# Kolkir/mono_slam_framework

Hardware: AMD Instinct MI355X
Metric: frame-pairs/sec (extract+match) (higher is better)
Workload: dtype u8; 1 GPU; ORB extract+match, 1280x720 pairs, 1024 pairs/GPU/step resident in HBM, ratio 0.60; pairs_per_gpu=1024, width=1280, height=720, synth_mode=0, overflow_pairs=0, ranks=1, rccl_ranks=0

## Files before the change

mono_slam_framework_amd/csrc/orb_kernels.hip:

```cpp
#include <type_traits>
#include "orb_pipeline.h"

#include <math.h>
#include <stdlib.h>
#include <string.h>

#include "orb_pattern.h"

namespace msf {

constexpr int SW = TW + 2, SH = TH + 2;
constexpr int kTileCandCap = TW * TH / 4;
constexpr int kTileY0 = kEdge;

constexpr uint32_t kStatusOverflow = 1u;

__constant__ __attribute__((aligned(16))) signed char c_pattern[1024];
__constant__ uint32_t c_disc[2 * kDiscTasks];

__device__ __forceinline__ __amdgpu_buffer_rsrc_t uniform_rsrc(const void* p, uint32_t bytes) {
  const unsigned long long v = (unsigned long long)p;
  const uint32_t lo = (uint32_t)__builtin_amdgcn_readfirstlane((int)(uint32_t)v);
  const uint32_t hi = (uint32_t)__builtin_amdgcn_readfirstlane((int)(uint32_t)(v >> 32));
  return __builtin_amdgcn_make_buffer_rsrc((void*)(((unsigned long long)hi << 32) | lo), 0,
                                           (int)__builtin_amdgcn_readfirstlane((int)bytes), 0x00020000);
}
__device__ __forceinline__ uint32_t uniform_u32(uint32_t v) { return (uint32_t)__builtin_amdgcn_readfirstlane((int)v); }
__device__ __forceinline__ const uint8_t* level_ptr(const OrbGeometry& g, const FrameSrc& src,
                                                    const uint8_t* pyr, int fi, int l, int* pitch) {
  if (l == 0) {
    *pitch = src.row_stride;
    return fi < src.n_a ? src.a + (long long)fi * src.frame_stride
                        : src.b + (long long)(fi - src.n_a) * src.frame_stride;
  }
  *pitch = g.lv[l].pitch;
  return pyr + (long long)(src.slot0 + fi) * g.pyr_bytes + g.lv[l].pix_off;
}

typedef unsigned short us2_t __attribute__((ext_vector_type(2)));
__device__ __forceinline__ uint32_t udot2_u16(uint32_t a, uint32_t b, uint32_t c) {
  return __builtin_amdgcn_udot2(__builtin_bit_cast(us2_t, a), __builtin_bit_cast(us2_t, b), c, false);
}

__device__ __forceinline__ uint32_t mad_u24(uint32_t a, uint32_t b, uint32_t c) {
  uint32_t r;
  asm("v_mad_u32_u24 %0, %1, %2, %3" : "=v"(r) : "v"(a), "v"(b), "v"(c));
  return r;
}

__device__ __forceinline__ uint32_t mad_u24_s(uint32_t a, uint32_t b_uniform, uint32_t c) {
  uint32_t r;
  asm("v_mad_u32_u24 %0, %1, %2, %3" : "=v"(r) : "v"(a), "s"(b_uniform), "v"(c));
  return r;
}

constexpr int kResizeMaxRows = 16;
template <bool SHARED>
__global__ __launch_bounds__(256) void k_resize(OrbGeometry g, FrameSrc src, uint8_t* pyr,
                                                const uint32_t* __restrict__ tab, int l, int rth, int lds_rows,
                                                uint32_t magic_n16, uint32_t magic_groups) {
  extern __shared__ __attribute__((aligned(16))) uint8_t smem[];
  uint32_t* ysh = reinterpret_cast<uint32_t*>(smem);
  uint8_t* rt = smem + 4 * kResizeMaxRows * 2;
  const int fi = blockIdx.y;
  const OrbLevelInfo L = g.lv[l];
  const int sh = g.lv[l - 1].h, sw16 = (g.lv[l - 1].w + 16 + 15) & ~15;
  int spitch;
  const uint8_t* s = level_ptr(g, src, pyr, fi, l - 1, &spitch);
  uint8_t* d = pyr + (long long)(src.slot0 + fi) * g.pyr_bytes + L.pix_off;
  const int groups = (L.w + 3) >> 2;
  const uint4* xsel = reinterpret_cast<const uint4*>(tab + L.tab_off);
  const uint4* xwxp = xsel + groups;
  const uint4* xoff = xwxp + groups;
  const uint32_t* ytab = reinterpret_cast<const uint32_t*>(xoff + groups);
  const int Y0 = blockIdx.x * rth, tid = threadIdx.x, nthr = blockDim.x;
  const int ylast = min(Y0 + rth, L.h) - 1;
  const int sy0 = ytab[Y0] & 0xFFFF;
  const int nrow = min((int)(ytab[ylast] & 0xFFFF) + 2 - sy0, lds_rows);
  const int n16 = sw16 >> 4, n4 = sw16 >> 2, rows = ylast - Y0 + 1;
  const int rowb = 4 * n4;
  if (tid < kResizeMaxRows) {
    const int y = Y0 + min(tid, rows - 1);
    const uint32_t yt = ytab[y];
    const uint32_t step1 = (tid > 0 && tid < rows && (yt & 0xFFFF) == (ytab[y - 1] & 0xFFFF) + 1u) ? 0x80000000u : 0u;
    ysh[2 * tid] = (uint32_t)(((int)(yt & 0xFFFF) - sy0) * rowb);
    ysh[2 * tid + 1] = (yt >> 16) | step1;
  }
  const int rgs = (rows + 3) >> 2, ntask = rgs * groups;
  int i = tid;
  int rg = magic_groups ? (int)__umulhi((uint32_t)min(i, ntask - 1), magic_groups) : min(i, ntask - 1);
  int gq = min(i, ntask - 1) - rg * groups;
  uint4 qs = xsel[gq], qw = xwxp[gq], qo = xoff[gq];
  for (int i = tid; i < nrow * n16; i += nthr) {
    const int r = (int)__umulhi((uint32_t)i, magic_n16), c = i - r * n16;
    const int gx = 16 * c, gy = sy0 + r;
    uint4 v = make_uint4(0u, 0u, 0u, 0u);
    if (gy < sh && gx + 16 <= spitch) v = *reinterpret_cast<const uint4*>(s + (long long)gy * spitch + gx);
    reinterpret_cast<uint4*>(rt)[i] = v;
  }
  __syncthreads();
  for (; i < ntask; i += nthr) {
    const int x4 = 4 * gq, ry0 = 4 * rg;
    const uint32_t sel[4] = {qs.x, qs.y, qs.z, qs.w}, wxp[4] = {qw.x, qw.y, qw.z, qw.w};
    const uint32_t boff[4] = {qo.x + (uint32_t)rowb, (SHARED ? qo.x : qo.y) + (uint32_t)rowb,
                              (SHARED ? qo.x : qo.z) + (uint32_t)rowb, qo.w + (uint32_t)rowb};
    {
      const int in = min(i + nthr, ntask - 1);
      rg = magic_groups ? (int)__umulhi((uint32_t)in, magic_groups) : in;
      gq = in - rg * groups;
      qs = xsel[gq], qw = xwxp[gq], qo = xoff[gq];
    }
    const char* Tb = reinterpret_cast<const char*>(rt);
    uint8_t* dp = d + (long long)(Y0 + ry0) * L.pitch + x4;
    const uint4 ya = *reinterpret_cast<const uint4*>(ysh + 2 * ry0), yb = *reinterpret_cast<const uint4*>(ysh + 2 * ry0 + 4);
    const uint32_t yrb[4] = {ya.x, ya.z, yb.x, yb.z}, ywy[4] = {ya.y, ya.w, yb.y, yb.w};
    uint32_t hlow[4];
#pragma unroll
    for (int j = 0; j < 4; j++) {
      const char* pr = Tb + yrb[j];
      if (j == 0 || (int)ywy[j] >= 0) {
#pragma unroll
        for (int k = 0; k < 4; k++) {
          const uint32_t* pa = reinterpret_cast<const uint32_t*>(pr + boff[k] - rowb);
          hlow[k] = udot2_u16(__builtin_amdgcn_perm(pa[1], pa[0], sel[k]), wxp[k], 0u);
        }
      }
      const uint32_t wy1 = ywy[j], wy0 = 256u - wy1;
      uint32_t v[4];
#pragma unroll
      for (int k = 0; k < 4; k++) {
        const uint32_t* pc = reinterpret_cast<const uint32_t*>(pr + boff[k]);
        const uint32_t h1 = udot2_u16(__builtin_amdgcn_perm(pc[1], pc[0], sel[k]), wxp[k], 0u);
        v[k] = mad_u24(hlow[k], wy0, mad_u24(h1, wy1, 32768u));
        hlow[k] = h1;
      }
      const uint32_t packed = __builtin_amdgcn_perm(v[1], v[0], 0x0c0c0602u) | __builtin_amdgcn_perm(v[3], v[2], 0x06020c0cu);
      if (ry0 + j < rows) *reinterpret_cast<uint32_t*>(dp) = packed;
      dp += L.pitch;
    }
  }
}

constexpr int HX = 16, HY = 4;
constexpr int PW2 = TW + 2 * HX, PH2 = TH + 2 * HY;
constexpr int SCO = 4;
constexpr int GPR = TW / 4 + 2;
constexpr int kList1Cap = 2 * SW * SH;
static_assert(kFastT % 2 == 0, "prefilter constants assume an even FAST threshold (cv::ORB default 20)");

__device__ __forceinline__ uint32_t mbcnt64(unsigned long long m) {
  return __builtin_amdgcn_mbcnt_hi((uint32_t)(m >> 32), __builtin_amdgcn_mbcnt_lo((uint32_t)m, 0u));
}

template <bool BRIGHT, int PITCH = PW2>
__device__ __forceinline__ int fast_score_pol(const uint8_t* p, int tau) {
  constexpr int off[16] = {3 * PITCH + 0,  3 * PITCH + 1,  2 * PITCH + 2,  1 * PITCH + 3,  0 * PITCH + 3, -1 * PITCH + 3,
                           -2 * PITCH + 2, -3 * PITCH + 1, -3 * PITCH + 0, -3 * PITCH - 1, -2 * PITCH - 2, -1 * PITCH - 3,
                           0 * PITCH - 3,  1 * PITCH - 3,  2 * PITCH - 2,  3 * PITCH - 1};
  int q[16];
// ... 1244 lines not shown
                                                     const uint32_t* __restrict__ s1_cnt, uint4* s1) {
  const int fi = blockIdx.y, slot = src.slot0 + fi, lane = threadIdx.x & 63;
  const int u = blockIdx.x * 4 + (threadIdx.x >> 6);
  if (u >= hw.base[g.nlevels]) return;
  int l = 0;
#pragma unroll
  for (int i = 1; i < kOrbLevels; i++)
    if (i < g.nlevels && u >= hw.base[i]) l = i;
  const OrbLevelInfo L = g.lv[l];
  const uint32_t kept = min(s1_cnt[slot * kOrbLevels + l], (uint32_t)kS1Cap);
  uint4* out = s1 + (long long)slot * g.s1_total + L.s1_off;
  int pitch;
  const uint8_t* img = level_ptr(g, src, pyr, fi, l, &pitch);
  const uint32_t step = 64u * (uint32_t)hw.n[l];
  for (uint32_t i = 64u * (uint32_t)(u - hw.base[l]) + lane; i < kept; i += step) {
    const uint32_t key = out[i].x;
    out[i].y = __float_as_uint(harris_at(img, pitch, key & 0xFFFF, key >> 16));
  }
}

constexpr int kSelCap = kKpCap;
__global__ __launch_bounds__(256) void k_select(OrbGeometry g, int slot0, const uint32_t* s1_cnt, const uint4* s1,
                                                msf_keypoint* kp, uint32_t* kp_cnt, uint32_t* status) {
  __shared__ uint4 kept[kSelCap];
  constexpr int kRespCap = 4096;
  __shared__ __attribute__((aligned(16))) float resp[kRespCap];
  __shared__ __attribute__((aligned(16))) uint32_t keys[kSelCap];
  __shared__ uint32_t nkept;
  const int slot = slot0 + blockIdx.x, tid = threadIdx.x;
  msf_keypoint* out = kp + (long long)slot * kKpCap;
  uint32_t base = 0;
  bool overflow = false;
  for (int l = 0; l < g.nlevels; l++) {
    const OrbLevelInfo L = g.lv[l];
    const uint32_t n = s1_cnt[slot * kOrbLevels + l];
    const uint4* in = s1 + (long long)slot * g.s1_total + L.s1_off;
    const uint32_t keep = (uint32_t)L.quota;
    if (tid == 0) nkept = 0;
    const bool staged = n > keep && n <= (uint32_t)kRespCap;
    const uint32_t n4 = (n + 3) >> 2;
    if (staged)
      for (uint32_t i = tid; i < 4 * n4; i += 256) resp[i] = i < n ? __uint_as_float(in[i].y) : -INFINITY;
    __syncthreads();
    for (uint32_t i = tid; i < n; i += 256) {
      const uint4 e = in[i];
      bool k = true;
      if (n > keep) {
        const float v = __uint_as_float(e.y);
        uint32_t greater = 0;
        if (staged) {
          const float4* r4 = reinterpret_cast<const float4*>(resp);
          for (uint32_t j = 0; j < n4; j++) {
            const float4 r = r4[j];
            greater += (uint32_t)(r.x > v) + (uint32_t)(r.y > v) + (uint32_t)(r.z > v) + (uint32_t)(r.w > v);
          }
        } else {
          for (uint32_t j = 0; j < n; j++) greater += (__uint_as_float(in[j].y) > v) ? 1u : 0u;
        }
        k = greater < keep;
      }
      if (k) {
        const uint32_t q = atomicAdd(&nkept, 1u);
        if (q < (uint32_t)kSelCap) kept[q] = e;
      }
    }
    __syncthreads();
    uint32_t m = nkept;
    if (m > (uint32_t)kSelCap) { overflow = true; m = kSelCap; }
    if (base + m > (uint32_t)kKpCap) { overflow = true; m = kKpCap - base; }
    const uint32_t m4 = (m + 3) >> 2;
    for (uint32_t i = tid; i < 4 * m4; i += 256) keys[i] = i < m ? kept[i].x : 0xFFFFFFFFu;
    __syncthreads();
    for (uint32_t i = tid; i < m; i += 256) {
      const uint4 e = kept[i];
      uint32_t rank = 0;
      const uint4* k4 = reinterpret_cast<const uint4*>(keys);
      for (uint32_t j = 0; j < m4; j++) {
        const uint4 kk = k4[j];
        rank += (uint32_t)(kk.x < e.x) + (uint32_t)(kk.y < e.x) + (uint32_t)(kk.z < e.x) + (uint32_t)(kk.w < e.x);
      }
      msf_keypoint k;
      k.lx = e.x & 0xFFFF;
      k.ly = e.x >> 16;
      k.x = (float)k.lx * L.scale;
      k.y = (float)k.ly * L.scale;
      k.response = __uint_as_float(e.y);
      k.angle = -1.f;
      k.octave = l;
      k.fast_score = (int)e.z;
      out[base + rank] = k;
    }
    base += m;
    __syncthreads();
  }
  if (tid == 0) {
    kp_cnt[slot] = base;
    if (overflow) atomicOr(&status[slot], kStatusOverflow);
  }
}

__device__ __forceinline__ float fast_atan2_deg(float y, float x) {
  const float k = (float)(180.0 / 3.14159265358979323846);
  const float p1 = 0.9997878412794807f * k, p3 = -0.3258083974640975f * k, p5 = 0.1555786518463281f * k,
              p7 = -0.04432655554792128f * k;
  const float ax = fabsf(x), ay = fabsf(y);
  float a, c, c2;
  if (ax >= ay) {
    c = ay / (ax + (float)2.2204460492503131e-16);
    c2 = c * c;
    a = (((p7 * c2 + p5) * c2 + p3) * c2 + p1) * c;
  } else {
    c = ax / (ay + (float)2.2204460492503131e-16);
    c2 = c * c;
    a = 90.f - (((p7 * c2 + p5) * c2 + p3) * c2 + p1) * c;
  }
  if (x < 0) a = 180.f - a;
  if (y < 0) a = 360.f - a;
  return a;
}

__device__ __forceinline__ void det_sincosf(float t, float* s, float* c) {
  const double x = (double)t;
  const int k = (int)(x * 6.36619772367581382433e-01 + 0.5);
  const double kd = (double)k;
  const double r = (x - kd * 1.57079632673412561417e+00) - kd * 6.07710050650619224932e-11;
  const double z = r * r;
  double p = 1.58969099521155010221e-10;
  p = p * z + -2.50507602534068634195e-08;
  p = p * z + 2.75573137070700676789e-06;
  p = p * z + -1.98412698298579493134e-04;
  p = p * z + 8.33333333332248946124e-03;
  p = p * z + -1.66666666666666324348e-01;
  const double sr = r + (r * z) * p;
  double q = -1.13596475577881948265e-11;
  q = q * z + 2.08757232129817482790e-09;
  q = q * z + -2.75573143513906633035e-07;
  q = q * z + 2.48015872894767294178e-05;
  q = q * z + -1.38888888888741095749e-03;
  q = q * z + 4.16666666666666019037e-02;
  const double cr = (1.0 - 0.5 * z) + (z * z) * q;
  double sv, cv;
  switch (k & 3) {
    case 0: sv = sr; cv = cr; break;
    case 1: sv = cr; cv = -sr; break;
    case 2: sv = -sr; cv = -cr; break;
    default: sv = -cr; cv = sr; break;
  }
  *s = (float)sv;
  *c = (float)cv;
}

constexpr int PR = 22;
constexpr int PD = 2 * PR + 1;
constexpr int PP = 48;
constexpr int HP = 40;
constexpr int HC = 46;

template <bool HALF_UP, bool SUM256>
__global__ __launch_bounds__(256) void k_describe(OrbGeometry g, FrameSrc src, const uint8_t* pyr,
                                                  msf_keypoint* kp, const uint32_t* kp_cnt, uint8_t* desc) {
  __shared__ __attribute__((aligned(16))) uint8_t raw_s[4][PD * PP + 16];
  __shared__ __attribute__((aligned(16))) uint16_t hb_s[4][HP * HC];
  __shared__ uint32_t disc_s[2 * kDiscTasks];
  __shared__ __attribute__((aligned(16))) int pat_s[256];
  const int fi = blockIdx.y, slot = src.slot0 + fi;
  const int wave = __builtin_amdgcn_readfirstlane((int)(threadIdx.x >> 6)), lane = threadIdx.x & 63;
  for (int i = threadIdx.x; i < 2 * kDiscTasks; i += 256) disc_s[i] = c_disc[i];
  pat_s[threadIdx.x] = reinterpret_cast<const int*>(c_pattern)[threadIdx.x];
  __shared__ unsigned long long lvl_base_s[kOrbLevels];
  __shared__ int lvl_pitch_s[kOrbLevels];
  if (threadIdx.x < kOrbLevels) {
    int pt = 0;
    const uint8_t* bp = level_ptr(g, src, pyr, fi, threadIdx.x < g.nlevels ? (int)threadIdx.x : 0, &pt);
    lvl_base_s[threadIdx.x] = (unsigned long long)bp;
    lvl_pitch_s[threadIdx.x] = pt;
  }
  __syncthreads();
  const uint32_t count = min(kp_cnt[slot], (uint32_t)kKpCap);
  uint8_t* raw = raw_s[wave];
  uint16_t* hb = hb_s[wave];
  uint32_t* raw32 = reinterpret_cast<uint32_t*>(raw);
  constexpr int NPL = (PD * (PP / 4) + 63) / 64;
  const uint32_t kstride = gridDim.x * 4;
  uint32_t k = blockIdx.x * 4 + wave;
  uint32_t pre[NPL];
  int xo_pre = 0;
  auto meta = [&](uint32_t k_) -> uint3 {
    if (k_ >= count) return make_uint3(0u, 0u, 0u);
    const msf_keypoint* Kp = kp + (long long)slot * kKpCap + k_;
    return make_uint3((uint32_t)Kp->octave, (uint32_t)Kp->lx, (uint32_t)Kp->ly);
  };
  auto issue = [&](uint3 m) {
    const uint32_t lv = (uint32_t)__builtin_amdgcn_readfirstlane((int)m.x);
    const int mx = __builtin_amdgcn_readfirstlane((int)m.y), my = __builtin_amdgcn_readfirstlane((int)m.z);
    const uint32_t pitch_ = (uint32_t)__builtin_amdgcn_readfirstlane(lvl_pitch_s[lv]);
    const unsigned long long b64 = lvl_base_s[lv];
    const unsigned long long img_ = ((unsigned long long)(uint32_t)__builtin_amdgcn_readfirstlane((int)(b64 >> 32)) << 32) |
                                    (uint32_t)__builtin_amdgcn_readfirstlane((int)(uint32_t)b64);
    typedef const __attribute__((address_space(1))) uint8_t* gptr_t;
    const int ax = (mx - PR) & ~3;
    xo_pre = (mx - PR) - ax;
    gptr_t base = (gptr_t)(img_ + (unsigned long long)((long long)(my - PR) * (long long)pitch_ + ax));
    const uint32_t pm = pitch_ - (uint32_t)PP;
#pragma unroll
    for (int u = 0; u < NPL; u++) {
      const uint32_t i = (uint32_t)lane + 64u * (uint32_t)u;
      const uint32_t r = (i * 43691u) >> 19;
      const uint32_t off = mad_u24(r, pm, 4u * i);
      pre[u] = i < (uint32_t)(PD * (PP / 4)) ? *(const __attribute__((address_space(1))) uint32_t*)(base + off) : 0u;
    }
  };
  uint32_t* hb32 = reinterpret_cast<uint32_t*>(hb);
  const int blur_rl = (lane * 26) >> 8, blur_gq = lane - 10 * blur_rl;
  const int blur_rd = blur_rl * (2 * (PP / 4)) + blur_gq, blur_wr = blur_gq * (4 * (HC / 2)) + blur_rl;
  const bool blur_last = 18 + blur_rl < 23;
  const uint32_t samp_base = (uint32_t)(uintptr_t)(__attribute__((address_space(3))) uint16_t*)hb +
                             2u * (uint32_t)((PR - 3) * HC + (PR - 3)) - 2u * HC * 0x400000u - 2u * 0x4B400000u;
  uint3 m_cur = meta(k), m_next = meta(k + kstride);
  if (k < count) issue(m_cur);
  for (; k < count; k += kstride) {
    const bool active = true;
    msf_keypoint* K = kp + (long long)slot * kKpCap + k;
    const int l = (int)m_cur.x, cx = (int)m_cur.y, cy = (int)m_cur.z;
    (void)l; (void)cx; (void)cy;
    const int xo = xo_pre;
#pragma unroll
    for (int u = 0; u < NPL; u++) {
      const int i = lane + 64 * u;
      if (i < PD * (PP / 4)) raw32[i] = pre[u];
    }
    m_cur = m_next;
    if (k + kstride < count) issue(m_cur);
    m_next = meta(k + 2 * kstride);
    MSF_WAVE_SYNC();
    float angle = 0.f;
    if (active) {
      int m10 = 0, m01 = 0;
      {
        const int dw0 = 1 + ((xo + 2) >> 2);
        const uint32_t shf = (uint32_t)(xo + 2) & 3u;
#pragma unroll
        for (int it = 0; it < kDiscTasks / 64; it++) {
          const int t = it * 64 + lane;
          const int row = t >> 3, k = t & 7;
          const uint32_t* d = raw32 + (row + 7) * (PP / 4) + dw0 + k;
          const uint32_t pxw = __builtin_amdgcn_alignbyte(d[1], d[0], shf) ^ 0x80808080u;
          const uint32_t wu = disc_s[2 * t], wv = disc_s[2 * t + 1];
          m10 = __builtin_amdgcn_sdot4((int)pxw, (int)wu, m10, false);
          m01 = __builtin_amdgcn_sdot4((int)pxw, (int)wv, m01, false);
        }
      }
      m10 = (int)__builtin_amdgcn_readlane((int)wave_incl_scan((uint32_t)m10), 63);
      m01 = (int)__builtin_amdgcn_readlane((int)wave_incl_scan((uint32_t)m01), 63);
      angle = fast_atan2_deg((float)m01, (float)m10);
      {
        constexpr uint32_t T0 = 18, T1 = 34, T2 = SUM256 ? 48 : 49, T3 = SUM256 ? 56 : 55;
        constexpr uint32_t A0 = T0 | T1 << 8 | T2 << 16 | T3 << 24, B0 = T2 | T1 << 8 | T0 << 16;
        constexpr uint32_t A1 = T0 << 8 | T1 << 16 | T2 << 24, B1 = T3 | T2 << 8 | T1 << 16 | T0 << 24;
        constexpr uint32_t A2 = T0 << 16 | T1 << 24, B2 = T2 | T3 << 8 | T2 << 16 | T1 << 24, C2 = T0;
        constexpr uint32_t A3 = T0 << 24, B3 = T1 | T2 << 8 | T3 << 16 | T2 << 24, C3 = T1 | T0 << 8;
        auto row4 = [&](const uint32_t* d, uint32_t* o) {
          const uint32_t d0 = d[0], d1 = d[1], d2 = d[2], d3 = d[3];
          const uint32_t e0 = __builtin_amdgcn_alignbyte(d1, d0, xo), e1 = __builtin_amdgcn_alignbyte(d2, d1, xo);
          const uint32_t e2 = __builtin_amdgcn_alignbyte(d3, d2, xo);
          o[0] = __builtin_amdgcn_udot4(e0, A0, __builtin_amdgcn_udot4(e1, B0, 0u, false), false);
          o[1] = __builtin_amdgcn_udot4(e0, A1, __builtin_amdgcn_udot4(e1, B1, 0u, false), false);
          o[2] = __builtin_amdgcn_udot4(e0, A2, __builtin_amdgcn_udot4(e1, B2, __builtin_amdgcn_udot4(e2, C2, 0u, false), false), false);
          o[3] = __builtin_amdgcn_udot4(e0, A3, __builtin_amdgcn_udot4(e1, B3, __builtin_amdgcn_udot4(e2, C3, 0u, false), false), false);
        };
#pragma unroll
        for (int it = 0; it < 4; it++) {
          const uint32_t* d = raw32 + blur_rd + it * (12 * (PP / 4));
          uint32_t ou[4], ol[4];
          row4(d, ou);
          row4(d + PP / 4, ol);
          if (it < 3 || blur_last) {
            uint32_t* w = hb32 + blur_wr + it * 6;
#pragma unroll
            for (int j = 0; j < 4; j++) w[j * (HC / 2)] = ou[j] | (ol[j] << 16);
          }
        }
      }
    }
    MSF_WAVE_SYNC();
    if (active) {
      float a, b;
      float rad = angle;
      rad *= (float)(3.14159265358979323846 / 180.f);
      det_sincosf(rad, &b, &a);
      const int4 pk = *reinterpret_cast<const int4*>(&pat_s[lane * 4]);
      const int words[4] = {pk.x, pk.y, pk.z, pk.w};
      uint32_t nib = 0;
      constexpr uint32_t K2 = SUM256 ? 48 : 49, K3 = SUM256 ? 56 : 55;
      constexpr uint32_t P0 = 18u | 34u << 16, P1 = K2 | K3 << 16, P2 = K2 | 34u << 16, P3 = 18u;
#pragma unroll
      for (int t = 0; t < 4; t++) {
        uint32_t val[2];
#pragma unroll
        for (int e = 0; e < 2; e++) {
          const float px = (float)(signed char)(words[t] >> (16 * e));
          const float py = (float)(signed char)(words[t] >> (16 * e + 8));
          const uint32_t tx = __float_as_uint((px * a - py * b) + 12582912.f);
          const uint32_t ty = __float_as_uint((px * b + py * a) + 12582912.f);
          const uint32_t addr = mad_u24(tx, 2u * HC, (ty << 1) + samp_base);
          const __attribute__((address_space(3))) uint32_t* q =
              (const __attribute__((address_space(3))) uint32_t*)(uintptr_t)(addr & ~3u);
          const uint32_t sh = addr & 2u;
          const uint32_t d0 = q[0], d1 = q[1], d2 = q[2], d3 = q[3];
          const uint32_t w0 = __builtin_amdgcn_alignbyte(d1, d0, sh), w1 = __builtin_amdgcn_alignbyte(d2, d1, sh);
          const uint32_t w2 = __builtin_amdgcn_alignbyte(d3, d2, sh), w3 = __builtin_amdgcn_alignbyte(0u, d3, sh);
          const uint32_t sum = udot2_u16(w0, P0, udot2_u16(w1, P1, udot2_u16(w2, P2, udot2_u16(w3, P3, 0u))));
          const uint32_t r = HALF_UP ? (sum + 32768u) >> 16 : (sum + 0x7FFFu + ((sum >> 16) & 1u)) >> 16;
          val[e] = min(r, 255u);
        }
        nib |= (uint32_t)(val[0] < val[1]) << t;
      }
      const uint32_t hi = __shfl_down(nib, 1);
      if ((lane & 1) == 0) desc[((long long)slot * kKpCap + k) * 32 + (lane >> 1)] = (uint8_t)(nib | (hi << 4));
      if (lane == 0) K->angle = angle;
    }
    MSF_WAVE_SYNC();
  }
}

constexpr int kTrainChunk = 1024;
__global__ __launch_bounds__(256) void k_match(int n_pairs, const int32_t* slot_a, const int32_t* slot_b,
                                               const msf_keypoint* kp, const uint32_t* kp_cnt, const uint8_t* desc,
                                               const uint32_t* status, float ratio, msf_match* out, int cap,
                                               int32_t* n_out, int chunk, int slot_base, int max_slots) {
  __shared__ __attribute__((aligned(16))) unsigned long long train[kTrainChunk * 4];
  __shared__ uint32_t wave_cnt[4];
  __shared__ uint32_t running;
  const int pair = blockIdx.x, tid = threadIdx.x, lane = tid & 63, wave = tid >> 6;
  const int sa = slot_a ? slot_a[pair] : slot_base + pair;
  const int sb = slot_b ? slot_b[pair] : slot_base + n_pairs + pair;
  if (sa < 0 || sa >= max_slots || sb < 0 || sb >= max_slots || ((status[sa] | status[sb]) & kStatusOverflow)) {
    if (tid == 0) n_out[pair] = -1;
    return;
  }
  const uint32_t n1 = min(kp_cnt[sa], (uint32_t)kKpCap), n2 = min(kp_cnt[sb], (uint32_t)kKpCap);
  const unsigned long long* tsrc = reinterpret_cast<const unsigned long long*>(desc + (long long)sb * kKpCap * 32);
  if (tid == 0) running = 0;
  __syncthreads();
  const msf_keypoint* ka = kp + (long long)sa * kKpCap;
  const msf_keypoint* kb = kp + (long long)sb * kKpCap;
  msf_match* o = out + (long long)pair * cap;
  for (uint32_t q0 = 0; q0 < n1; q0 += 256) {
    const uint32_t q = q0 + tid;
    const bool have_q = q < n1;
    unsigned long long q0w = 0, q1w = 0, q2w = 0, q3w = 0;
    if (have_q) {
      const unsigned long long* qd =
          reinterpret_cast<const unsigned long long*>(desc + ((long long)sa * kKpCap + q) * 32);
      q0w = qd[0]; q1w = qd[1]; q2w = qd[2]; q3w = qd[3];
    }
    int d0 = 0x7fffffff, d1 = 0x7fffffff, i0 = -1;
    for (uint32_t t0 = 0; t0 < n2; t0 += chunk) {
      const uint32_t tn = min(n2 - t0, (uint32_t)chunk);
      __syncthreads();
      for (uint32_t i = tid; i < tn * 4; i += 256) train[i] = tsrc[(size_t)t0 * 4 + i];
      __syncthreads();
      if (have_q) {
        for (uint32_t t = 0; t < tn; t++) {
          const unsigned long long* tr = &train[t * 4];
          const int d = __popcll(q0w ^ tr[0]) + __popcll(q1w ^ tr[1]) + __popcll(q2w ^ tr[2]) + __popcll(q3w ^ tr[3]);
          if (d < d1) {
            if (d < d0) { d1 = d0; d0 = d; i0 = (int)(t0 + t); }
            else d1 = d;
          }
        }
      }
    }
    const bool pass = have_q && n2 >= 2 && ((float)d0 < ratio * (float)d1);
    const unsigned long long bal = __ballot(pass);
    const uint32_t before = __popcll(bal & ((1ull << lane) - 1ull));
    if (lane == 0) wave_cnt[wave] = __popcll(bal);
    __syncthreads();
    uint32_t off = running;
    for (int w = 0; w < wave; w++) off += wave_cnt[w];
    if (pass) {
      const uint32_t idx = off + before;
      if (idx < (uint32_t)cap) {
        msf_match m;
        m.x1 = (int)ka[q].x; m.y1 = (int)ka[q].y;
        m.x2 = (int)kb[i0].x; m.y2 = (int)kb[i0].y;
        o[idx] = m;
      }
    }
    __syncthreads();
    if (tid == 0) running += wave_cnt[0] + wave_cnt[1] + wave_cnt[2] + wave_cnt[3];
    __syncthreads();
  }
  if (tid == 0) n_out[pair] = (int32_t)running;
}

constexpr int kSplitBlocks = kKpCap / 64;
constexpr int kSplitMaxPairs = 128;
__global__ __launch_bounds__(256) void k_match_split(int n_pairs, const int32_t* slot_a, const int32_t* slot_b,
                                                     const msf_keypoint* kp, const uint32_t* kp_cnt,
                                                     const uint8_t* desc, const uint32_t* status, float ratio,
                                                     msf_match* out, int cap, int32_t* n_out, int chunk,
                                                     uint32_t* qres, uint32_t* done, int slot_base, int max_slots) {
  __shared__ __attribute__((aligned(16))) unsigned long long train[kTrainChunk * 4];
  __shared__ int part[3][4][64];
  __shared__ uint32_t wave_cnt[4];
  __shared__ uint32_t running, last_s;
  const int pair = blockIdx.y, qb = blockIdx.x, tid = threadIdx.x, lane = tid & 63, wave = tid >> 6;
  const int sa = slot_a ? slot_a[pair] : slot_base + pair;
  const int sb = slot_b ? slot_b[pair] : slot_base + n_pairs + pair;
  if (sa < 0 || sa >= max_slots || sb < 0 || sb >= max_slots || ((status[sa] | status[sb]) & kStatusOverflow)) {
    if (qb == 0 && tid == 0) n_out[pair] = -1;
    return;
  }
  const uint32_t n1 = min(kp_cnt[sa], (uint32_t)kKpCap), n2 = min(kp_cnt[sb], (uint32_t)kKpCap);
  const unsigned long long* tsrc = reinterpret_cast<const unsigned long long*>(desc + (long long)sb * kKpCap * 32);
  uint32_t* qr = qres + (long long)pair * kKpCap;
  const uint32_t q = (uint32_t)qb * 64u + lane;
  if ((uint32_t)qb * 64u < n1) {
    const bool have_q = q < n1;
    unsigned long long q0w = 0, q1w = 0, q2w = 0, q3w = 0;
    if (have_q) {
      const unsigned long long* qd = reinterpret_cast<const unsigned long long*>(desc + ((long long)sa * kKpCap + q) * 32);
      q0w = qd[0]; q1w = qd[1]; q2w = qd[2]; q3w = qd[3];
    }
    int d0 = 0x7fffffff, d1 = 0x7fffffff, i0 = 0x7fffffff;
    for (uint32_t t0 = 0; t0 < n2; t0 += chunk) {
      const uint32_t tn = min(n2 - t0, (uint32_t)chunk);
      __syncthreads();
      for (uint32_t i = tid; i < tn * 4; i += 256) train[i] = tsrc[(size_t)t0 * 4 + i];
      __syncthreads();
      const uint32_t ta = (tn * wave) >> 2, tb = (tn * (wave + 1)) >> 2;
      for (uint32_t t = ta; t < tb; t++) {
// ... 614 lines not shown
```

Baseline: 165,000 frame-pairs/sec.

## Compute descriptor patch row blur with MFMA int8 tiles and remap block-to-frame

```diff
diff --git a/mono_slam_framework_amd/csrc/orb_blur_tiles.h b/mono_slam_framework_amd/csrc/orb_blur_tiles.h
--- /dev/null
+++ b/mono_slam_framework_amd/csrc/orb_blur_tiles.h
@@ -0,0 +1,85 @@
+#pragma once
+#include <stdint.h>
+
+namespace msf {
+namespace blur_tiles {
+
+constexpr int kRawPitch = 48;
+constexpr int kRawRows = 45;
+constexpr int kRawRowsRead = 48;
+constexpr int kRawBytes = kRawRowsRead * kRawPitch + 16;
+constexpr int kFetchLoads = 9;
+constexpr int kFetchLanes = 60;
+constexpr int kHbCols = 40;
+constexpr int kHbRows = 46;
+constexpr int kHbPitch = 52;
+constexpr int kHbEntries = kHbCols * kHbPitch;
+constexpr int kTilesM = 3, kTilesN = 3;
+
+constexpr int tap(bool sum256, int j) {
+  const int k = j < 4 ? j : 6 - j;
+  return k == 0 ? 18 : k == 1 ? 34 : k == 2 ? (sum256 ? 48 : 49) : (sum256 ? 56 : 55);
+}
+constexpr int acc_init(bool sum256) { return 128 * (sum256 ? 256 : 257); }
+
+constexpr int fetch_lane(int lane) { return lane < kFetchLanes ? lane : kFetchLanes - 1; }
+constexpr int fetch_row(int lane) { return fetch_lane(lane) / 12; }
+constexpr int fetch_dword(int lane) { return fetch_lane(lane) % 12; }
+constexpr int raw_dword_of_load(int u, int lane) { return 60 * u + fetch_lane(lane); }
+
+constexpr int raw_col(int group, int byte) { return 16 * group + byte; }
+constexpr int a_byte_offset(int mt, int lane) { return (16 * mt + lane % 16) * kRawPitch + 16 * (lane / 16); }
+constexpr int b_weight(bool sum256, int nt, int lane, int byte) {
+  const int k = raw_col(lane / 16, byte), j = k - (16 * nt + lane % 16) - 2;
+  return k < kRawPitch && j >= 0 && j < 7 ? tap(sum256, j) : 0;
+}
+constexpr uint64_t tap_word(bool sum256) {
+  return (uint64_t)tap(sum256, 0) | (uint64_t)tap(sum256, 1) << 8 | (uint64_t)tap(sum256, 2) << 16 | (uint64_t)tap(sum256, 3) << 24 |
+         (uint64_t)tap(sum256, 4) << 32 | (uint64_t)tap(sum256, 5) << 40 | (uint64_t)tap(sum256, 6) << 48;
+}
+constexpr uint32_t b_dword(bool sum256, int nt, int lane, int d) {
+  const int j0 = 16 * (lane / 16) + 4 * d - (16 * nt + lane % 16) - 2;
+  return lane >= 48 || j0 <= -4 || j0 >= 7 ? 0u
+         : j0 >= 0 ? (uint32_t)(tap_word(sum256) >> (8 * j0)) : (uint32_t)(tap_word(sum256) << (8 * -j0));
+}
+
+constexpr int d_col(int nt, int lane) { return 16 * nt + lane % 16; }
+constexpr int d_row0(int mt, int lane) { return 16 * mt + 4 * (lane / 16); }
+constexpr int hb_store_dwords(int mt, int nt, int lane) {
+  return d_col(nt, lane) >= kHbCols ? 0 : d_row0(mt, lane) + 4 <= kHbRows ? 2 : d_row0(mt, lane) + 2 <= kHbRows ? 1 : 0;
+}
+constexpr int hb_store_byte_offset(int mt, int nt, int lane) { return 2 * (d_col(nt, lane) * kHbPitch + d_row0(mt, lane)); }
+constexpr uint32_t pack2(uint32_t lo, uint32_t hi) { return (lo & 0xFFFFu) | hi << 16; }
+
+constexpr int moment_dword(int t) { return (7 + t / 8) * (kRawPitch / 4) + 2 + t % 8; }
+constexpr int kSampleReach = 19;
+constexpr int samp_byte_offset(int ix, int iy) { return 2 * ((kSampleReach + ix) * kHbPitch + kSampleReach + iy); }
+
+inline void model_row_blur(bool sum256, const uint8_t* raw, uint16_t* hb) {
+  for (int mt = 0; mt < kTilesM; mt++)
+    for (int nt = 0; nt < kTilesN; nt++) {
+      int32_t acc[16][16];
+      for (int i = 0; i < 16; i++)
+        for (int n = 0; n < 16; n++) acc[i][n] = acc_init(sum256);
+      for (int la = 0; la < 64; la++)
+        for (int lb = 0; lb < 64; lb++) {
+          if (la / 16 != lb / 16) continue;
+          const uint8_t* a = raw + a_byte_offset(mt, la);
+          for (int j = 0; j < 16; j++)
+            acc[la % 16][lb % 16] += (int32_t)(int8_t)a[j] * (int32_t)(int8_t)(b_dword(sum256, nt, lb, j / 4) >> (8 * (j % 4)));
+        }
+      for (int lane = 0; lane < 64; lane++) {
+        const int n = hb_store_dwords(mt, nt, lane);
+        uint16_t* w = hb + hb_store_byte_offset(mt, nt, lane) / 2;
+        const int i0 = d_row0(mt, lane) - 16 * mt, c = lane % 16;
+        for (int i = 0; i < n; i++) {
+          const uint32_t pair = pack2((uint32_t)acc[i0 + 2 * i][c], (uint32_t)acc[i0 + 2 * i + 1][c]);
+          w[2 * i] = (uint16_t)pair;
+          w[2 * i + 1] = (uint16_t)(pair >> 16);
+        }
+      }
+    }
+}
+
+}
+}
diff --git a/mono_slam_framework_amd/csrc/orb_kernels.hip b/mono_slam_framework_amd/csrc/orb_kernels.hip
--- a/mono_slam_framework_amd/csrc/orb_kernels.hip
+++ b/mono_slam_framework_amd/csrc/orb_kernels.hip
@@ -5,6 +5,7 @@
 #include <stdlib.h>
 #include <string.h>
 
+#include "orb_blur_tiles.h"
 #include "orb_pattern.h"
 
 namespace msf {
@@ -1555,18 +1556,25 @@
 
 constexpr int PR = 22;
 constexpr int PD = 2 * PR + 1;
-constexpr int PP = 48;
-constexpr int HP = 40;
-constexpr int HC = 46;
+constexpr int PP = blur_tiles::kRawPitch;
+constexpr int HP = blur_tiles::kHbCols;
+constexpr int HC = blur_tiles::kHbPitch;
+static_assert(PD == blur_tiles::kRawRows && PD * (PP / 4) == blur_tiles::kFetchLoads * blur_tiles::kFetchLanes, "patch fetch");
+typedef int v4i_t __attribute__((ext_vector_type(4)));
 
 template <bool HALF_UP, bool SUM256>
 __global__ __launch_bounds__(256) void k_describe(OrbGeometry g, FrameSrc src, const uint8_t* pyr,
                                                   msf_keypoint* kp, const uint32_t* kp_cnt, uint8_t* desc) {
-  __shared__ __attribute__((aligned(16))) uint8_t raw_s[4][PD * PP + 16];
-  __shared__ __attribute__((aligned(16))) uint16_t hb_s[4][HP * HC];
+  __shared__ __attribute__((aligned(16))) uint8_t raw_s[4][blur_tiles::kRawBytes];
+  __shared__ __attribute__((aligned(16))) uint16_t hb_s[4][blur_tiles::kHbEntries];
   __shared__ uint32_t disc_s[2 * kDiscTasks];
   __shared__ __attribute__((aligned(16))) int pat_s[256];
-  const int fi = blockIdx.y, slot = src.slot0 + fi;
+  int fi = blockIdx.y, part = blockIdx.x;
+  if (gridDim.x == 8 && (fi | 7) < (int)gridDim.y) {
+    part = fi & 7;
+    fi = (fi & ~7) | (int)blockIdx.x;
+  }
+  const int slot = src.slot0 + fi;
   const int wave = __builtin_amdgcn_readfirstlane((int)(threadIdx.x >> 6)), lane = threadIdx.x & 63;
   for (int i = threadIdx.x; i < 2 * kDiscTasks; i += 256) disc_s[i] = c_disc[i];
   pat_s[threadIdx.x] = reinterpret_cast<const int*>(c_pattern)[threadIdx.x];
@@ -1583,16 +1591,17 @@
   uint8_t* raw = raw_s[wave];
   uint16_t* hb = hb_s[wave];
   uint32_t* raw32 = reinterpret_cast<uint32_t*>(raw);
-  constexpr int NPL = (PD * (PP / 4) + 63) / 64;
+  constexpr int NPL = blur_tiles::kFetchLoads;
   const uint32_t kstride = gridDim.x * 4;
-  uint32_t k = blockIdx.x * 4 + wave;
+  uint32_t k = (uint32_t)part * 4 + wave;
   uint32_t pre[NPL];
-  int xo_pre = 0;
   auto meta = [&](uint32_t k_) -> uint3 {
     if (k_ >= count) return make_uint3(0u, 0u, 0u);
     const msf_keypoint* Kp = kp + (long long)slot * kKpCap + k_;
     return make_uint3((uint32_t)Kp->octave, (uint32_t)Kp->lx, (uint32_t)Kp->ly);
   };
+  const int fl = blur_tiles::fetch_lane(lane);
+  const uint32_t fetch_row = (uint32_t)blur_tiles::fetch_row(lane), fetch_x4 = 4u * (uint32_t)blur_tiles::fetch_dword(lane);
   auto issue = [&](uint3 m) {
     const uint32_t lv = (uint32_t)__builtin_amdgcn_readfirstlane((int)m.x);
     const int mx = __builtin_amdgcn_readfirstlane((int)m.y), my = __builtin_amdgcn_readfirstlane((int)m.z);
@@ -1601,24 +1610,25 @@
     const unsigned long long img_ = ((unsigned long long)(uint32_t)__builtin_amdgcn_readfirstlane((int)(b64 >> 32)) << 32) |
                                     (uint32_t)__builtin_amdgcn_readfirstlane((int)(uint32_t)b64);
     typedef const __attribute__((address_space(1))) uint8_t* gptr_t;
-    const int ax = (mx - PR) & ~3;
-    xo_pre = (mx - PR) - ax;
-    gptr_t base = (gptr_t)(img_ + (unsigned long long)((long long)(my - PR) * (long long)pitch_ + ax));
-    const uint32_t pm = pitch_ - (uint32_t)PP;
-#pragma unroll
-    for (int u = 0; u < NPL; u++) {
-      const uint32_t i = (uint32_t)lane + 64u * (uint32_t)u;
-      const uint32_t r = (i * 43691u) >> 19;
-      const uint32_t off = mad_u24(r, pm, 4u * i);
-      pre[u] = i < (uint32_t)(PD * (PP / 4)) ? *(const __attribute__((address_space(1))) uint32_t*)(base + off) : 0u;
-    }
+    const unsigned long long base = img_ + (unsigned long long)((long long)(my - PR) * (long long)pitch_ + (mx - PP / 2));
+    const uint32_t off = mad_u24(fetch_row, pitch_, fetch_x4);
+#pragma unroll
+    for (int u = 0; u < NPL; u++)
+      pre[u] = *(const __attribute__((address_space(1))) uint32_t*)((gptr_t)(base + (unsigned long long)(5u * (uint32_t)u * pitch_)) + off);
   };
-  uint32_t* hb32 = reinterpret_cast<uint32_t*>(hb);
-  const int blur_rl = (lane * 26) >> 8, blur_gq = lane - 10 * blur_rl;
-  const int blur_rd = blur_rl * (2 * (PP / 4)) + blur_gq, blur_wr = blur_gq * (4 * (HC / 2)) + blur_rl;
-  const bool blur_last = 18 + blur_rl < 23;
-  const uint32_t samp_base = (uint32_t)(uintptr_t)(__attribute__((address_space(3))) uint16_t*)hb +
-                             2u * (uint32_t)((PR - 3) * HC + (PR - 3)) - 2u * HC * 0x400000u - 2u * 0x4B400000u;
+  const uint32_t raw_lds = (uint32_t)(uintptr_t)(__attribute__((address_space(3))) uint8_t*)raw;
+  const uint32_t hb_lds = (uint32_t)(uintptr_t)(__attribute__((address_space(3))) uint16_t*)hb;
+  const uint32_t blur_a = (uint32_t)blur_tiles::a_byte_offset(0, lane);
+  const uint32_t blur_w = (uint32_t)blur_tiles::hb_store_byte_offset(0, 0, lane);
+  v4i_t blur_b[blur_tiles::kTilesN];
+#pragma unroll
+  for (int nt = 0; nt < blur_tiles::kTilesN; nt++)
+#pragma unroll
+    for (int d = 0; d < 4; d++) blur_b[nt][d] = (int)blur_tiles::b_dword(SUM256, nt, lane, d);
+  const bool blur_cols = (lane & 15) < HP - 32;
+  const bool blur_rows = (lane >> 4) < 3;
+  static_assert(blur_tiles::kSampleReach == PR - 3, "the blur's three taps on either side of the pattern's reach");
+  const uint32_t samp_base = hb_lds + (uint32_t)blur_tiles::samp_byte_offset(0, 0) - 2u * HC * 0x400000u - 2u * 0x4B400000u;
   uint3 m_cur = meta(k), m_next = meta(k + kstride);
   if (k < count) issue(m_cur);
   for (; k < count; k += kstride) {
@@ -1626,12 +1636,8 @@
     msf_keypoint* K = kp + (long long)slot * kKpCap + k;
     const int l = (int)m_cur.x, cx = (int)m_cur.y, cy = (int)m_cur.z;
     (void)l; (void)cx; (void)cy;
-    const int xo = xo_pre;
-#pragma unroll
-    for (int u = 0; u < NPL; u++) {
-      const int i = lane + 64 * u;
-      if (i < PD * (PP / 4)) raw32[i] = pre[u];
-    }
+#pragma unroll
+    for (int u = 0; u < NPL; u++) raw32[60 * u + fl] = pre[u] ^ 0x80808080u;
     m_cur = m_next;
     if (k + kstride < count) issue(m_cur);
     m_next = meta(k + 2 * kstride);
@@ -1640,14 +1646,11 @@
     if (active) {
       int m10 = 0, m01 = 0;
       {
-        const int dw0 = 1 + ((xo + 2) >> 2);
-        const uint32_t shf = (uint32_t)(xo + 2) & 3u;
 #pragma unroll
         for (int it = 0; it < kDiscTasks / 64; it++) {
           const int t = it * 64 + lane;
           const int row = t >> 3, k = t & 7;
-          const uint32_t* d = raw32 + (row + 7) * (PP / 4) + dw0 + k;
-          const uint32_t pxw = __builtin_amdgcn_alignbyte(d[1], d[0], shf) ^ 0x80808080u;
+          const uint32_t pxw = raw32[(row + 7) * (PP / 4) + 2 + k];
           const uint32_t wu = disc_s[2 * t], wv = disc_s[2 * t + 1];
           m10 = __builtin_amdgcn_sdot4((int)pxw, (int)wu, m10, false);
           m01 = __builtin_amdgcn_sdot4((int)pxw, (int)wv, m01, false);
@@ -1657,30 +1660,27 @@
       m01 = (int)__builtin_amdgcn_readlane((int)wave_incl_scan((uint32_t)m01), 63);
       angle = fast_atan2_deg((float)m01, (float)m10);
       {
-        constexpr uint32_t T0 = 18, T1 = 34, T2 = SUM256 ? 48 : 49, T3 = SUM256 ? 56 : 55;
-        constexpr uint32_t A0 = T0 | T1 << 8 | T2 << 16 | T3 << 24, B0 = T2 | T1 << 8 | T0 << 16;
-        constexpr uint32_t A1 = T0 << 8 | T1 << 16 | T2 << 24, B1 = T3 | T2 << 8 | T1 << 16 | T0 << 24;
-        constexpr uint32_t A2 = T0 << 16 | T1 << 24, B2 = T2 | T3 << 8 | T2 << 16 | T1 << 24, C2 = T0;
-        constexpr uint32_t A3 = T0 << 24, B3 = T1 | T2 << 8 | T3 << 16 | T2 << 24, C3 = T1 | T0 << 8;
-        auto row4 = [&](const uint32_t* d, uint32_t* o) {
-          const uint32_t d0 = d[0], d1 = d[1], d2 = d[2], d3 = d[3];
-          const uint32_t e0 = __builtin_amdgcn_alignbyte(d1, d0, xo), e1 = __builtin_amdgcn_alignbyte(d2, d1, xo);
-          const uint32_t e2 = __builtin_amdgcn_alignbyte(d3, d2, xo);
-          o[0] = __builtin_amdgcn_udot4(e0, A0, __builtin_amdgcn_udot4(e1, B0, 0u, false), false);
-          o[1] = __builtin_amdgcn_udot4(e0, A1, __builtin_amdgcn_udot4(e1, B1, 0u, false), false);
-          o[2] = __builtin_amdgcn_udot4(e0, A2, __builtin_amdgcn_udot4(e1, B2, __builtin_amdgcn_udot4(e2, C2, 0u, false), false), false);
-          o[3] = __builtin_amdgcn_udot4(e0, A3, __builtin_amdgcn_udot4(e1, B3, __builtin_amdgcn_udot4(e2, C3, 0u, false), false), false);
-        };
-#pragma unroll
-        for (int it = 0; it < 4; it++) {
-          const uint32_t* d = raw32 + blur_rd + it * (12 * (PP / 4));
-          uint32_t ou[4], ol[4];
-          row4(d, ou);
-          row4(d + PP / 4, ol);
-          if (it < 3 || blur_last) {
-            uint32_t* w = hb32 + blur_wr + it * 6;
-#pragma unroll
-            for (int j = 0; j < 4; j++) w[j * (HC / 2)] = ou[j] | (ol[j] << 16);
+        typedef __attribute__((address_space(3))) const v4i_t* lds_v4_t;
+        typedef uint32_t v2u_t __attribute__((ext_vector_type(2)));
+        typedef __attribute__((address_space(3))) v2u_t* lds_u2_t;
+        typedef __attribute__((address_space(3))) uint32_t* lds_u1_t;
+        constexpr int C0 = blur_tiles::acc_init(SUM256);
+        const v4i_t c0 = {C0, C0, C0, C0};
+#pragma unroll
+        for (int mt = 0; mt < blur_tiles::kTilesM; mt++) {
+          const v4i_t av = *(lds_v4_t)(uintptr_t)(raw_lds + blur_a + (uint32_t)(16 * mt * PP));
+#pragma unroll
+          for (int nt = 0; nt < blur_tiles::kTilesN; nt++) {
+            const v4i_t dv = __builtin_amdgcn_mfma_i32_16x16x64_i8(av, blur_b[nt], c0, 0, 0, 0);
+            const uint32_t wa = hb_lds + blur_w + (uint32_t)(2 * (16 * nt * HC + 16 * mt));
+            const uint32_t lo = __builtin_amdgcn_perm((uint32_t)dv[1], (uint32_t)dv[0], 0x05040100u);
+            const uint32_t hi = __builtin_amdgcn_perm((uint32_t)dv[3], (uint32_t)dv[2], 0x05040100u);
+            if (mt < 2) {
+              if (nt < 2 || blur_cols) *(lds_u2_t)(uintptr_t)wa = v2u_t{lo, hi};
+            } else if (nt < 2 || blur_cols) {
+              if (blur_rows) *(lds_u2_t)(uintptr_t)wa = v2u_t{lo, hi};
+              else *(lds_u1_t)(uintptr_t)wa = lo;
+            }
           }
         }
       }
```

Result: faster. 167,800 frame-pairs/sec (median of 6 runs) (+1.7%).
